# bupt-ai-cz/HIAST

Measured on AMD Instinct MI355X. Metric: self-training images/sec (fwd+bwd+pseudo-label) at 1024x512, higher is better.
Workload: dtype fp16

## Files before the change

### hiast_amd/csrc/xconv_bs.hip

```cpp
#include <hip/hip_bf16.h>
#include <stdlib.h>

#include "common.h"

namespace hiast {

typedef __attribute__((ext_vector_type(8))) __bf16 xb_bf16x8;
typedef __attribute__((ext_vector_type(4))) float xb_f32x4;
typedef __attribute__((address_space(3))) void* xb_lds_ptr;

constexpr int XB_PANEL = 64;
constexpr int XB_STAGES = 3;
constexpr int XB_COLS = 256;
constexpr int XB_KC = 256;

__device__ __forceinline__ void xb_dma16(__amdgpu_buffer_rsrc_t rs, unsigned char* lds, int voff, int soff)
{
    __builtin_amdgcn_raw_ptr_buffer_load_lds(rs, (xb_lds_ptr)lds, 16, voff, soff, 0, 0);
}
__device__ __forceinline__ int xb_lds_off(int row, int chunk) { return row * 128 + ((chunk ^ ((row >> 1) & 7)) << 4); }
template <int IDX>
__device__ __forceinline__ xb_bf16x8 xb_lds_read_i(unsigned addr)
{
    xb_bf16x8 v;
    asm volatile("ds_read_b128 %0, %1 offset:%2" : "=v"(v) : "v"(addr), "i"(IDX * 2048));
    return v;
}
__device__ __forceinline__ xb_bf16x8 xb_lds_read(unsigned addr, int idx)
{
    switch (idx) {
    case 1: return xb_lds_read_i<1>(addr);
    case 2: return xb_lds_read_i<2>(addr);
    case 3: return xb_lds_read_i<3>(addr);
    case 4: return xb_lds_read_i<4>(addr);
    case 5: return xb_lds_read_i<5>(addr);
    case 6: return xb_lds_read_i<6>(addr);
    case 7: return xb_lds_read_i<7>(addr);
    case 8: return xb_lds_read_i<8>(addr);
    case 9: return xb_lds_read_i<9>(addr);
    case 10: return xb_lds_read_i<10>(addr);
    case 11: return xb_lds_read_i<11>(addr);
    case 12: return xb_lds_read_i<12>(addr);
    case 13: return xb_lds_read_i<13>(addr);
    case 14: return xb_lds_read_i<14>(addr);
    case 15: return xb_lds_read_i<15>(addr);
    default: return xb_lds_read_i<0>(addr);
    }
}
__device__ __forceinline__ void xb_lds_wait(xb_bf16x8& a, xb_bf16x8& b)
{
    asm volatile("s_waitcnt lgkmcnt(0)" : "+v"(a), "+v"(b));
}

template <bool F16>
__global__ __launch_bounds__(512) void xconv_gated_bnstat_kernel(
    const unsigned short* __restrict__ X, const unsigned short* __restrict__ Wp, const unsigned short* __restrict__ R,
    const unsigned char* __restrict__ Rg, const unsigned short* __restrict__ BX, const unsigned char* __restrict__ BM,
    const float* __restrict__ bmean, const float* __restrict__ binvstd, unsigned short* __restrict__ Y, int M, int N,
    float* __restrict__ stats)
{
    constexpr int SL = XB_KC / 64;
    constexpr int KS = XB_KC / 32;
    constexpr int STAGE = XB_PANEL * XB_KC * 2;
    __shared__ __attribute__((aligned(1024))) unsigned char smem[XB_STAGES * STAGE];

    const int tid = threadIdx.x, lane = tid & 63;
    const int wave = __builtin_amdgcn_readfirstlane(tid >> 6);
    const int g = lane >> 4, px = lane & 15;
    const int NG = N / XB_COLS;
    const int xcd = blockIdx.x & 7, slot = blockIdx.x >> 3;
    const int cg = slot % NG;
    const int nstream = (int)gridDim.x / NG;
    const int stream = (slot / NG) * 8 + xcd;
    const int n0 = cg * XB_COLS + wave * 32;
    const int npanel = (M + XB_PANEL - 1) / XB_PANEL;
    const int c0 = n0 + g * 8;

    xb_bf16x8 wr[2][KS];
#pragma unroll
    for (int b = 0; b < 2; ++b) {
        const unsigned short* wrow = Wp + (size_t)(n0 + (px >> 2) * 8 + b * 4 + (px & 3)) * XB_KC + g * 8;
#pragma unroll
        for (int s = 0; s < KS; ++s) wr[b][s] = *reinterpret_cast<const xb_bf16x8*>(wrow + s * 32);
    }
#pragma unroll
    for (int b = 0; b < 2; ++b)
#pragma unroll
        for (int s = 0; s < KS; ++s) asm volatile("" : "+v"(wr[b][s]));

    constexpr int OOB = (int)0x80000000;
    const __amdgpu_buffer_rsrc_t xrs = __builtin_amdgcn_make_buffer_rsrc((void*)X, 0, (int)((size_t)M * XB_KC * 2), 0x00020000);
    const int drow = wave * 8 + (lane >> 3);
    const int dchunk = ((lane & 7) ^ ((drow >> 1) & 7)) * 16;
    auto issue = [&](int p, int st) {
        const int m = p * XB_PANEL + drow;
        const int voff = (p < npanel && m < M) ? (int)((size_t)m * XB_KC * 2) + dchunk : OOB;
        unsigned char* base = smem + st * STAGE + wave * 1024;
#pragma unroll
        for (int j = 0; j < SL; ++j) xb_dma16(xrs, base + j * (XB_PANEL * 128), voff, j * 128);
    };
    const unsigned lds_base = (unsigned)(size_t)smem;
    float st1[8], st2[8];
#pragma unroll
    for (int q = 0; q < 8; ++q) { st1[q] = 0.f; st2[q] = 0.f; }

    struct Rows {
        uint4 res[4], bx[4];
        unsigned gate[4], bm[4];
    };
    Rows ring[2];
    auto load_rows = [&](Rows& r, int p) {
#pragma unroll
        for (int t = 0; t < 4; ++t) {
            const int m = p * XB_PANEL + t * 16 + px;
            const size_t mr = (size_t)((p < npanel && m < M) ? m : 0);
            r.res[t] = h_load16_once(R + mr * N + c0);
            r.gate[t] = Rg[mr * (N >> 3) + (c0 >> 3)];
            r.bx[t] = h_load16_once(BX + mr * N + c0);
            r.bm[t] = BM[mr * (N >> 3) + (c0 >> 3)];
        }
    };
    auto panel = [&](int p, int it, const Rows& cur, Rows& nxt) {
        const int st = it % XB_STAGES;
        if (it == 0) asm volatile("s_waitcnt vmcnt(%0)\n\ts_barrier" ::"n"(SL + 16) : "memory");
        else asm volatile("s_waitcnt vmcnt(%0)\n\ts_barrier" ::"n"(SL + 4) : "memory");
        load_rows(nxt, p + nstream);
        issue(p + 2 * nstream, (it + 2) % XB_STAGES);
        const unsigned fbase = lds_base + (unsigned)(st * STAGE) + (unsigned)xb_lds_off(px, g);
#pragma unroll
        for (int half = 0; half < 2; ++half) {
            xb_f32x4 acc[2][2];
#pragma unroll
            for (int a = 0; a < 2; ++a)
#pragma unroll
                for (int b = 0; b < 2; ++b) acc[a][b] = (xb_f32x4){0.f, 0.f, 0.f, 0.f};
            auto frag = [&](int s, int a) {
                return xb_lds_read((s & 1) ? fbase ^ 64u : fbase, 4 * (s >> 1) + 2 * half + a);
            };
            xb_bf16x8 xa[2][2];
            xa[0][0] = frag(0, 0);
            xa[0][1] = frag(0, 1);
            xb_lds_wait(xa[0][0], xa[0][1]);
#pragma unroll
            for (int s = 0; s < KS; ++s) {
                if (s + 1 < KS) {
                    xa[(s + 1) & 1][0] = frag(s + 1, 0);
                    xa[(s + 1) & 1][1] = frag(s + 1, 1);
                }
#pragma unroll
                for (int a = 0; a < 2; ++a)
#pragma unroll
                    for (int b = 0; b < 2; ++b) acc[a][b] = H16<F16>::mfma16(wr[b][s], xa[s & 1][a], acc[a][b]);
                if (s + 1 < KS) xb_lds_wait(xa[(s + 1) & 1][0], xa[(s + 1) & 1][1]);
            }
#pragma unroll
            for (int a = 0; a < 2; ++a) {
                const int t = 2 * half + a;
                const int m = p * XB_PANEL + t * 16 + px;
                const bool ok = m < M;
                const unsigned w0[4] = {cur.res[t].x, cur.res[t].y, cur.res[t].z, cur.res[t].w};
                const unsigned xw[4] = {cur.bx[t].x, cur.bx[t].y, cur.bx[t].z, cur.bx[t].w};
                const unsigned gate = cur.gate[t], bm = cur.bm[t];
                unsigned pk[4];
#pragma unroll
                for (int q = 0; q < 4; ++q) {
                    float o0 = acc[a][q >> 1][2 * (q & 1)], o1 = acc[a][q >> 1][2 * (q & 1) + 1];
                    o0 += ((gate >> (2 * q)) & 1u) ? H16<F16>::lo(w0[q]) : 0.f;
                    o1 += ((gate >> (2 * q + 1)) & 1u) ? H16<F16>::hi(w0[q]) : 0.f;
                    pk[q] = H16<F16>::pack(o0, o1);
                    if (ok) {
                        const float g0 = ((bm >> (2 * q)) & 1u) ? H16<F16>::lo(pk[q]) : 0.f;
                        const float g1 = ((bm >> (2 * q + 1)) & 1u) ? H16<F16>::hi(pk[q]) : 0.f;
                        st1[2 * q] += g0;
                        st2[2 * q] = fmaf(g0, H16<F16>::lo(xw[q]), st2[2 * q]);
                        st1[2 * q + 1] += g1;
                        st2[2 * q + 1] = fmaf(g1, H16<F16>::hi(xw[q]), st2[2 * q + 1]);
                    }
                }
                if (ok) h_store16_out(Y + (size_t)m * N + c0, pk[0], pk[1], pk[2], pk[3]);
            }
        }
    };

    issue(stream, 0);
    issue(stream + nstream, 1);
    load_rows(ring[0], stream);
    for (int p = stream, it = 0; p < npanel; p += 2 * nstream, it += 2) {
        panel(p, it, ring[0], ring[1]);
        if (p + nstream >= npanel) break;
        panel(p + nstream, it + 1, ring[1], ring[0]);
    }
#pragma unroll
    for (int q = 0; q < 8; ++q) {
#pragma unroll
        for (int o = 1; o < 16; o <<= 1) {
            st1[q] += __shfl_xor(st1[q], o, 64);
            st2[q] += __shfl_xor(st2[q], o, 64);
        }
    }
    if (px == 0) {
        float* d = stats + ((size_t)stream * N + c0) * 2;
#pragma unroll
        for (int q = 0; q < 8; ++q) {
            const float mu = bmean[c0 + q], is = binvstd[c0 + q];
            d[2 * q] = st1[q];
            d[2 * q + 1] = is * (st2[q] - mu * st1[q]);
        }
    }
}

static int xb_blocks(int64_t M, int N)
{
    const int NG = N / XB_COLS;
    const long long npanel = (M + XB_PANEL - 1) / XB_PANEL;
    long long streams = hiast_grid_cus() / NG / 8 * 8;
    if (streams < 8) streams = 8;
    if (streams > npanel) streams = (npanel + 7) / 8 * 8;
    return (int)(streams * NG);
}

}

extern "C" int hiast_xconv_dgrad_gated_bn_stats_rows(int64_t M, int K, int N)
{
    if (M < 4096 || K != hiast::XB_KC || N % hiast::XB_COLS != 0 || N > 2048) return 0;
    return hiast::xb_blocks(M, N) / (N / hiast::XB_COLS);
}

extern "C" int hiast_xconv_dgrad_gated_bn_stats(const void* dy, const void* wpt, const void* res, const void* res_gate,
                                                const void* bn_x, const void* bn_mask, const float* save_mean,
                                                const float* save_invstd, void* dx, float* partial, int64_t M, int K, int N,
                                                int fmt, hiast_stream_t stream)
{
    if (fmt != HIAST_FMT_BF16 && fmt != HIAST_FMT_FP16) return HIAST_E_RANGE;
    if (!dy || !wpt || !res || !res_gate || !bn_x || !bn_mask || !save_mean || !save_invstd || !dx || !partial) return HIAST_E_ARG;
    if (hiast_xconv_dgrad_gated_bn_stats_rows(M, K, N) == 0) return HIAST_E_RANGE;
    if ((size_t)M * N * 2 >= (1ull << 40) || (size_t)M * K * 2 >= (1ull << 31)) return HIAST_E_RANGE;
    if ((((uintptr_t)dy) | ((uintptr_t)wpt) | ((uintptr_t)res) | ((uintptr_t)bn_x) | ((uintptr_t)dx) | ((uintptr_t)save_mean) |
         ((uintptr_t)save_invstd)) & 15)
        return HIAST_E_RANGE;
    const dim3 grid((unsigned)hiast::xb_blocks(M, N));
    hipStream_t st = (hipStream_t)stream;
    if (fmt == HIAST_FMT_FP16)
        hipLaunchKernelGGL(hiast::xconv_gated_bnstat_kernel<true>, grid, dim3(512), 0, st, (const unsigned short*)dy,
                           (const unsigned short*)wpt, (const unsigned short*)res, (const unsigned char*)res_gate,
                           (const unsigned short*)bn_x, (const unsigned char*)bn_mask, save_mean, save_invstd,
                           (unsigned short*)dx, (int)M, N, partial);
    else
        hipLaunchKernelGGL(hiast::xconv_gated_bnstat_kernel<false>, grid, dim3(512), 0, st, (const unsigned short*)dy,
                           (const unsigned short*)wpt, (const unsigned short*)res, (const unsigned char*)res_gate,
                           (const unsigned short*)bn_x, (const unsigned char*)bn_mask, save_mean, save_invstd,
                           (unsigned short*)dx, (int)M, N, partial);
    HIAST_CHECK_LAUNCH();
    return 0;
}
```

Before: 141.2.

## Exchange accumulator halves between paired waves so each lane stores 64-channel rows

Result: no change. 141.1 (-0.1%).

```diff
diff --git a/hiast_amd/csrc/xconv_bs.hip b/hiast_amd/csrc/xconv_bs.hip
--- a/hiast_amd/csrc/xconv_bs.hip
+++ b/hiast_amd/csrc/xconv_bs.hip
@@ -13,6 +13,7 @@
 constexpr int XB_STAGES = 3;
 constexpr int XB_COLS = 256;
 constexpr int XB_KC = 256;
+constexpr int XB_XCH = 4096;
 
 __device__ __forceinline__ void xb_dma16(__amdgpu_buffer_rsrc_t rs, unsigned char* lds, int voff, int soff)
 {
@@ -51,6 +52,25 @@
 {
     asm volatile("s_waitcnt lgkmcnt(0)" : "+v"(a), "+v"(b));
 }
+template <int OFF>
+__device__ __forceinline__ void xb_xch_write(unsigned addr, const xb_f32x4& v)
+{
+    asm volatile("ds_write_b128 %0, %1 offset:%2" ::"v"(addr), "v"(v), "i"(OFF) : "memory");
+}
+template <int OFF>
+__device__ __forceinline__ void xb_xch_read(unsigned addr, xb_f32x4& v)
+{
+    asm volatile("ds_read_b128 %0, %1 offset:%2" : "+v"(v) : "v"(addr), "i"(OFF) : "memory");
+}
+__device__ __forceinline__ void xb_acc_settle(xb_f32x4& a, xb_f32x4& b, xb_f32x4& c, xb_f32x4& d)
+{
+    asm volatile("s_nop 15" : "+v"(a), "+v"(b), "+v"(c), "+v"(d));
+}
+__device__ __forceinline__ void xb_acc_wait(xb_f32x4& a, xb_f32x4& b, xb_f32x4& c, xb_f32x4& d)
+{
+    asm volatile("s_waitcnt lgkmcnt(0)" : "+v"(a), "+v"(b), "+v"(c), "+v"(d));
+}
+__device__ __forceinline__ void xb_xch_barrier() { asm volatile("s_waitcnt lgkmcnt(0)\n\ts_barrier" ::: "memory"); }
 
 template <bool F16>
 __global__ __launch_bounds__(512) void xconv_gated_bnstat_kernel(
@@ -62,7 +82,7 @@
     constexpr int SL = XB_KC / 64;
     constexpr int KS = XB_KC / 32;
     constexpr int STAGE = XB_PANEL * XB_KC * 2;
-    __shared__ __attribute__((aligned(1024))) unsigned char smem[XB_STAGES * STAGE];
+    __shared__ __attribute__((aligned(1024))) unsigned char smem[XB_STAGES * STAGE + 8 * XB_XCH];
 
     const int tid = threadIdx.x, lane = tid & 63;
     const int wave = __builtin_amdgcn_readfirstlane(tid >> 6);
@@ -74,7 +94,10 @@
     const int stream = (slot / NG) * 8 + xcd;
     const int n0 = cg * XB_COLS + wave * 32;
     const int npanel = (M + XB_PANEL - 1) / XB_PANEL;
-    const int c0 = n0 + g * 8;
+    const int odd = wave & 1;
+    const int rpx = (px & 7) + 8 * odd;
+    const int c0 = cg * XB_COLS + (wave >> 1) * 64 + (g + 4 * (px >> 3)) * 8;
+    const bool giver = (px >> 3) != odd;
 
     xb_bf16x8 wr[2][KS];
 #pragma unroll
@@ -100,6 +123,8 @@
         for (int j = 0; j < SL; ++j) xb_dma16(xrs, base + j * (XB_PANEL * 128), voff, j * 128);
     };
     const unsigned lds_base = (unsigned)(size_t)smem;
+    const unsigned xslot = lds_base + (unsigned)(XB_STAGES * STAGE) + (unsigned)((g * 8 + (px & 7)) * 16);
+    const unsigned xmine = xslot + (unsigned)(wave * XB_XCH), xpeer = xslot + (unsigned)((wave ^ 1) * XB_XCH);
     float st1[8], st2[8];
 #pragma unroll
     for (int q = 0; q < 8; ++q) { st1[q] = 0.f; st2[q] = 0.f; }
@@ -112,7 +137,7 @@
     auto load_rows = [&](Rows& r, int p) {
 #pragma unroll
         for (int t = 0; t < 4; ++t) {
-            const int m = p * XB_PANEL + t * 16 + px;
+            const int m = p * XB_PANEL + t * 16 + rpx;
             const size_t mr = (size_t)((p < npanel && m < M) ? m : 0);
             r.res[t] = h_load16_once(R + mr * N + c0);
             r.gate[t] = Rg[mr * (N >> 3) + (c0 >> 3)];
@@ -153,10 +178,25 @@
                     for (int b = 0; b < 2; ++b) acc[a][b] = H16<F16>::mfma16(wr[b][s], xa[s & 1][a], acc[a][b]);
                 if (s + 1 < KS) xb_lds_wait(xa[(s + 1) & 1][0], xa[(s + 1) & 1][1]);
             }
+            xb_acc_settle(acc[0][0], acc[0][1], acc[1][0], acc[1][1]);
+            if (giver) {
+                xb_xch_write<0>(xmine + half * 2048, acc[0][0]);
+                xb_xch_write<512>(xmine + half * 2048, acc[0][1]);
+                xb_xch_write<1024>(xmine + half * 2048, acc[1][0]);
+                xb_xch_write<1536>(xmine + half * 2048, acc[1][1]);
+            }
+            xb_xch_barrier();
+            if (giver) {
+                xb_xch_read<0>(xpeer + half * 2048, acc[0][0]);
+                xb_xch_read<512>(xpeer + half * 2048, acc[0][1]);
+                xb_xch_read<1024>(xpeer + half * 2048, acc[1][0]);
+                xb_xch_read<1536>(xpeer + half * 2048, acc[1][1]);
+            }
+            xb_acc_wait(acc[0][0], acc[0][1], acc[1][0], acc[1][1]);
 #pragma unroll
             for (int a = 0; a < 2; ++a) {
                 const int t = 2 * half + a;
-                const int m = p * XB_PANEL + t * 16 + px;
+                const int m = p * XB_PANEL + t * 16 + rpx;
                 const bool ok = m < M;
                 const unsigned w0[4] = {cur.res[t].x, cur.res[t].y, cur.res[t].z, cur.res[t].w};
                 const unsigned xw[4] = {cur.bx[t].x, cur.bx[t].y, cur.bx[t].z, cur.bx[t].w};
@@ -193,12 +233,41 @@
 #pragma unroll
     for (int q = 0; q < 8; ++q) {
 #pragma unroll
-        for (int o = 1; o < 16; o <<= 1) {
+        for (int o = 1; o < 8; o <<= 1) {
             st1[q] += __shfl_xor(st1[q], o, 64);
             st2[q] += __shfl_xor(st2[q], o, 64);
         }
     }
-    if (px == 0) {
+    {
+        xb_f32x4 lo1 = {st1[0], st1[1], st1[2], st1[3]}, hi1 = {st1[4], st1[5], st1[6], st1[7]};
+        xb_f32x4 lo2 = {st2[0], st2[1], st2[2], st2[3]}, hi2 = {st2[4], st2[5], st2[6], st2[7]};
+        const unsigned fin = (unsigned)((px >> 3) * 2048);
+        xb_xch_barrier();
+        if (odd) {
+            xb_xch_write<0>(xmine + fin, lo1);
+            xb_xch_write<512>(xmine + fin, hi1);
+            xb_xch_write<1024>(xmine + fin, lo2);
+            xb_xch_write<1536>(xmine + fin, hi2);
+        }
+        xb_xch_barrier();
+        if (!odd) {
+            xb_xch_read<0>(xpeer + fin, lo1);
+            xb_xch_read<512>(xpeer + fin, hi1);
+            xb_xch_read<1024>(xpeer + fin, lo2);
+            xb_xch_read<1536>(xpeer + fin, hi2);
+        }
+        xb_acc_wait(lo1, hi1, lo2, hi2);
+        if (!odd) {
+#pragma unroll
+            for (int q = 0; q < 4; ++q) {
+                st1[q] += lo1[q];
+                st1[q + 4] += hi1[q];
+                st2[q] += lo2[q];
+                st2[q + 4] += hi2[q];
+            }
+        }
+    }
+    if (!odd && (px & 7) == 0) {
         float* d = stats + ((size_t)stream * N + c0) * 2;
 #pragma unroll
         for (int q = 0; q < 8; ++q) {
```
